# xmlyqing00/V-FloodNet

Hardware: AMD Instinct MI355X
Metric: segmented frames/sec at 480p (higher is better)
Workload: dtype f32

## Files before the change

include/vfn_hip.h:

```cpp
#ifndef VFN_HIP_H
#define VFN_HIP_H

#ifdef __cplusplus
extern "C" {
#endif

#define VFN_ABI_VERSION 16
enum { VFN_DESC_CONV = 0, VFN_DESC_STEM = 1, VFN_DESC_BANKSCAN = 2, VFN_DESC_MEMREAD = 3, VFN_DESC_BANK = 4, VFN_DESC_WGRAD = 5,
       VFN_DESC_REFRESH_FILTER = 6, VFN_DESC_REFRESH_EPILOGUE = 7, VFN_DESC_GATHER = 8, VFN_DESC_BANKMATCH = 9,
       VFN_DESC_TRAIN_AUG = 10 };
int vfn_abi_version(void);
int vfn_sizeof_desc(int which);

typedef struct vfn_conv_desc {
    const float* in;
    const float* w;
    const float* scale;
    const float* shift;
    const float* res;
    float* out;
    int N, H, W, Cin, in_ld;
    int Ho, Wo, Cout, cout_pad, out_ld, res_ld;
    int KH, KW, stride, pad;
    int relu_in, relu_out;
    int M;
    int ksplit;
    int split_from;
    int res_mod;
    float* partial;
    int* tile_counters;
    int w_packed;
    int in_lp;
    int out_lp_relu;
    void* out_lp;
    const float* mask;
    int mask_ld;
    int mask_after;
    int w_batch_rows;
    int k_rot;
} vfn_conv_desc;

int vfn_conv_cfg_count(void);
int vfn_conv_cfg_tile(int cfg, int* bm, int* bn);
int vfn_conv_cfg_info(int cfg, int* bm, int* bn, int* wm, int* wn, int* dma);
int vfn_conv_cfg_modes(int cfg);
int vfn_conv_cfg_wk(int cfg);
int vfn_conv_cfg_tpb(int cfg);
#define VFN_CONV_SK_WS_FLOATS (16 * 1024 * 1024)
#define VFN_CONV_SK_MAX_TILES 16384
int vfn_conv_cfg_kind(int cfg);
int vfn_conv_cfg_name(int cfg, char* buf, int n);
int vfn_conv2d_nhwc_f32(const vfn_conv_desc* d, int cfg, void* stream);
int vfn_conv2d_nhwc_bf16(const vfn_conv_desc* d, int cfg, void* stream);
int vfn_conv2d_nhwc_bf16x3(const vfn_conv_desc* d, int cfg, void* stream);

int vfn_winograd_tiles(int N, int H, int W);
int vfn_winograd_input_f32(const float* x, int N, int H, int W, int C, int ld_x, int relu, float* V, int rows_pad, void* stream);
int vfn_winograd_output_f32(const float* Mb, int rows_pad, int N, int H, int W, int Cout, const float* scale, const float* shift,
                            const float* res, int res_ld, int res_mod, int relu_out, float* out, int out_ld, void* stream);
int vfn_winograd_output_masked_f32(const float* Mb, int rows_pad, int N, int H, int W, int Cout, const float* res, int res_ld,
                                   const float* mask, int mask_ld, int mask_after, float* out, int out_ld, void* stream);
int vfn_winograd_gemm_f32(const float* V, const float* U, float* Mb, int comps, int rows_pad, int C, int Cout, int cout_pad, int cfg,
                          int wgs, void* stream);
int vfn_conv1x1_persistent_f32(const vfn_conv_desc* d, int cfg, int wgs, void* stream);
int vfn_winograd_input_bf16(const float* x, int N, int H, int W, int C, int ld_x, int relu, void* V, int rows_pad, void* stream);
int vfn_winograd_gemm_bf16(const void* V, const void* U, float* Mb, int comps, int rows_pad, int C, int Cout, int cout_pad, int cfg,
                           int wgs, void* stream);
int vfn_winograd_gy_f32(const float* gy, int N, int H, int W, int C, int ld, float* Z, int rows_pad, void* stream);
int vfn_winograd_dw_f32(const float* dU, int Cout, int Cin, const float* rowscale, float* dw, int accumulate, void* stream);

typedef struct vfn_stem_desc {
    const float* frame;
    const float* mask;
    const float* w;
    const float* scale;
    const float* shift;
    float* out;
    float mean[3];
    float std[3];
    int N, cin;
    int H0, W0;
    int pad_top, pad_left;
    int Hp, Wp;
    int Ho, Wo;
} vfn_stem_desc;

int vfn_stem_conv7x7_f32(const vfn_stem_desc* d, void* stream);
int vfn_maxpool3x3s2_nhwc_f32(const float* in, float* out, int N, int H, int W, int C, void* stream);

int vfn_upsample2x_add_nhwc_f32(const float* s, const float* pm, float* out, int N, int h, int w, int C,
                                int s_bcast, void* stream);
int vfn_upsample2x_add_lp_nhwc_f32(const float* s, const float* pm, float* out, void* out_lp, int lp_relu,
// ... 310 lines not shown
```

v-floodnet_amd/_lib.py:

```python
import ctypes as C
import os

import torch

_HERE = os.path.dirname(os.path.abspath(__file__))
LIB_PATH = os.environ.get('VFN_LIB_PATH') or os.path.join(_HERE, 'libvfn_hip.so')

_lib = None

c_fp = C.c_void_p


class ConvDesc(C.Structure):
    _fields_ = [('inp', c_fp), ('w', c_fp), ('scale', c_fp), ('shift', c_fp), ('res', c_fp), ('out', c_fp),
                ('N', C.c_int), ('H', C.c_int), ('W', C.c_int), ('Cin', C.c_int), ('in_ld', C.c_int),
                ('Ho', C.c_int), ('Wo', C.c_int), ('Cout', C.c_int), ('cout_pad', C.c_int),
                ('out_ld', C.c_int), ('res_ld', C.c_int),
                ('KH', C.c_int), ('KW', C.c_int), ('stride', C.c_int), ('pad', C.c_int),
                ('relu_in', C.c_int), ('relu_out', C.c_int), ('M', C.c_int), ('ksplit', C.c_int),
                ('split_from', C.c_int), ('res_mod', C.c_int), ('partial', c_fp), ('tile_counters', c_fp),
                ('w_packed', C.c_int), ('in_lp', C.c_int), ('out_lp_relu', C.c_int), ('out_lp', c_fp), ('mask', c_fp), ('mask_ld', C.c_int), ('mask_after', C.c_int), ('w_batch_rows', C.c_int), ('k_rot', C.c_int)]


class WgradDesc(C.Structure):
# ... 58 lines not shown
class BankDesc(C.Structure):
    _fields_ = [('bank_k', c_fp), ('bank_v', c_fp), ('info', c_fp),
                ('scratch_k', c_fp), ('scratch_v', c_fp), ('scratch_info', c_fp),
                ('bank_len', c_fp), ('bank_len_rw', c_fp), ('bank_knorm', c_fp), ('bank_vnorm', c_fp),
                ('match_idx', c_fp), ('match_corr', c_fp), ('new_k', c_fp), ('new_knorm', c_fp), ('new_vnorm', c_fp),
                ('app_pos', c_fp), ('keep_dst', c_fp), ('plan', c_fp), ('stats', c_fp),
                ('stride_k', C.c_longlong), ('stride_v', C.c_longlong), ('stride_info', C.c_longlong),
                ('stride_n', C.c_longlong), ('stride_new', C.c_longlong),
                ('class_budget', C.c_double),
                ('thres_close', C.c_float), ('update_rate', C.c_float), ('new_hit_init', C.c_float),
                ('frame_idx', C.c_int), ('ld_new', C.c_int), ('voff', C.c_int), ('HW', C.c_int),
                ('obj_n', C.c_int), ('cap', C.c_int), ('rm_class', C.c_int), ('rm_request', C.c_int)]


class TrainAugFrame(C.Structure):
    _fields_ = [('m', C.c_double * 6), ('brightness', C.c_float), ('contrast', C.c_float), ('saturation', C.c_float),
                ('hue_shift', C.c_int), ('order', C.c_int * 4),
                ('flip', C.c_int), ('jitter', C.c_int), ('affine', C.c_int), ('nearest_tables', C.c_int),
                ('win_i', C.c_int), ('win_j', C.c_int), ('win_h', C.c_int), ('win_w', C.c_int)]


TRAIN_AUG_MAX_T, TRAIN_AUG_MAX_SIDE, TRAIN_AUG_MAX_OUT, TRAIN_AUG_MAX_OBJ = 16, 8192, 4096, 11


class TrainAugDesc(C.Structure):
    _fields_ = [('src', c_fp), ('mask', c_fp), ('jit', c_fp), ('lsum', c_fp), ('win_img', c_fp), ('win_mask', c_fp),
                ('aff_xtab', c_fp), ('aff_ytab', c_fp), ('hpass', c_fp), ('kx_bounds', c_fp), ('kx', c_fp),
                ('ky_bounds', c_fp), ('ky', c_fp), ('nx', c_fp), ('ny', c_fp), ('frames', c_fp), ('masks', c_fp),
                ('H', C.c_int), ('W', C.c_int), ('T', C.c_int), ('S', C.c_int), ('ksize_x', C.c_int), ('ksize_y', C.c_int),
                ('obj_n', C.c_int), ('obj_list', C.c_int * (TRAIN_AUG_MAX_OBJ - 1)),
                ('frame', TrainAugFrame * TRAIN_AUG_MAX_T)]


ABI_VERSION = 16
DESC_IDS = {0: ConvDesc, 1: StemDesc, 2: BankScanDesc, 3: MemReadDesc, 4: BankDesc, 5: WgradDesc, 6: RefreshFilter, 7: RefreshEpilogue, 8: GatherEntry, 9: BankMatchDesc, 10: TrainAugDesc}


def lib():
    global _lib
    if _lib is None:
        if not os.path.isfile(LIB_PATH):
            raise RuntimeError(
                f'{LIB_PATH} not found: build the HIP kernels first '
                '(python -c "import __graft_entry__ as g; g.build()" or make -C v-floodnet_amd/csrc)')
        L = C.CDLL(LIB_PATH)
        L.vfn_abi_version.restype = C.c_int
        if L.vfn_abi_version() != ABI_VERSION:
            raise RuntimeError(f'{LIB_PATH} has ABI version {L.vfn_abi_version()}, this package expects {ABI_VERSION} '
                               '(descriptor layouts differ): rebuild it (make -C v-floodnet_amd/csrc)')
        L.vfn_sizeof_desc.restype = C.c_int
        for which, cls in DESC_IDS.items():
            if L.vfn_sizeof_desc(which) != C.sizeof(cls):
                raise RuntimeError(f'{LIB_PATH}: sizeof({cls.__name__}) is {L.vfn_sizeof_desc(which)} in the library, '
                                   f'{C.sizeof(cls)} in this binding: rebuild it (make -C v-floodnet_amd/csrc)')
        _declare(L)
        _lib = L
    return _lib


def _declare(L):
    i, f, p = C.c_int, C.c_float, C.c_void_p
    L.vfn_abi_version.restype = i
    L.vfn_conv_cfg_count.restype = i
    L.vfn_conv_cfg_tile.argtypes = [i, C.POINTER(i), C.POINTER(i)]
    L.vfn_conv_cfg_info.argtypes = [i] + [C.POINTER(i)] * 5
    L.vfn_conv_cfg_wk.argtypes = [i]
    L.vfn_conv_cfg_wk.restype = i
# ... 35 lines not shown
_ll = C.c_longlong
SIGNATURES = {
    'vfn_maxpool3x3s2_nhwc_f32': [_p, _p, _i, _i, _i, _i, _p],
    'vfn_upsample2x_add_nhwc_f32': [_p, _p, _p, _i, _i, _i, _i, _i, _p],
    'vfn_upsample2x_add_lp_nhwc_f32': [_p, _p, _p, _p, _i, _i, _i, _i, _i, _i, _p],
    'vfn_rough_uncertainty_f32': [_p, _p, _p, _p, _i, _i, _i, _p],
    'vfn_transpose_taps_f32': [_p, _i, _i, _i, _i, _i, _i, _i, _i, _i, _i, _i, _p, _p, _i, _p],
    'vfn_dilate2_f32': [_p, _p, _i, _i, _i, _i, _i, _i, _p],
    'vfn_bn_param_grads_f32': [_p, _p, _p, _p, _p, _i, _i, _p, _i, _p, _p, _p],
    'vfn_bn_param_grads_acc_f32': [_p, _p, _p, _p, _p, _i, _i, _p, _i, _p, _p, _i, _p, _p],
    'vfn_maxpool3x3s2_backward_f32': [_p, _p, _p, _i, _i, _i, _i, _p, _i, _p],
    'vfn_softmax_cols_f32': [_p, _i, _i, _i, _f, _p, _p],
    'vfn_softmax_cols_backward_f32': [_p, _p, _i, _i, _i, _f, _p, _p],
    'vfn_adamw_f32': [_p, _p, _p, _p, _ll, C.c_double, C.c_double, C.c_double, C.c_double, C.c_double, _i, _p],
    'vfn_colsum_f32': [_p, _i, _i, _i, _p, _i, _p, _p],
    'vfn_colsum_acc_f32': [_p, _i, _i, _i, _p, _i, _p, _i, _p, _p],
    'vfn_upsample2x_add_backward_f32': [_p, _p, _p, _i, _i, _i, _i, _i, _p],
    'vfn_tail_grad_o_f32': [_p, _p, _p, _p, _p, _p, _i, _i, _i, _i, _i, _i, _i, _p],
    'vfn_segment_loss_f32': [_p, _p, _i, _i, _i, _f, _p, _p, _p, _p],
    'vfn_segment_uncertainty_backward_f32': [_p, _i, _i, _i, _p, _p, _p, _p, _p, _p],
    'vfn_tail_split_f32': [_p, _p, _p, _p, _p, _p, _p, _i, _i, _p],
    'vfn_local_stats_backward_f32': [_p] * 13 + [_i, _i, _i, _i, _p],
    'vfn_local_hpass_f32': [_p, _p, _p, _p, _p, _i, _i, _i, _i, _p],
    'vfn_local_vpass_f32': [_p, _p, _p, _p, _p, _i, _i, _i, _i, _p],
    'vfn_local_stats_f32': [_p, _p, _p, _p, _i, _i, _i, _i, _p],
    'vfn_pred2_gather_f32': [_p, _p, _p, _i, _i, _i, _i, _p],
    'vfn_final_logits_f32': [_p, _p, _p, _p, _p, _i, _i, _i, _i, _i, _i, _i, _p],
    'vfn_bank_scan_finish': [_p, _i, _i, _i, _i, _p, _p, _p, _p, _p],
    'vfn_row_norms': [_p, _ll, _i, _i, _p, _i, _i, _p, _p, _ll, _p],
    'vfn_scatter_mean_f32': [_p, _ll, _ll, _p, _i, _p, _ll, _ll, _i, _p],
    'vfn_winograd_tiles': [_i, _i, _i],
    'vfn_winograd_input_f32': [_p, _i, _i, _i, _i, _i, _i, _p, _i, _p],
    'vfn_winograd_output_f32': [_p, _i, _i, _i, _i, _i, _p, _p, _p, _i, _i, _i, _p, _i, _p],
    'vfn_winograd_gy_f32': [_p, _i, _i, _i, _i, _i, _p, _i, _p],
    'vfn_winograd_gemm_f32': [_p, _p, _p, _i, _i, _i, _i, _i, _i, _i, _p],
    'vfn_conv1x1_persistent_f32': [_p, _i, _i, _p],
    'vfn_winograd_input_bf16': [_p, _i, _i, _i, _i, _i, _i, _p, _i, _p],
    'vfn_winograd_gemm_bf16': [_p, _p, _p, _i, _i, _i, _i, _i, _i, _i, _p],
    'vfn_winograd_dw_f32': [_p, _i, _i, _p, _p, _i, _p],
    'vfn_winograd_output_masked_f32': [_p, _i, _i, _i, _i, _i, _p, _i, _p, _i, _i, _p, _i, _p],
    'vfn_scatter_mean_checked_f32': [_p, _ll, _ll, _p, _ll, _i, _p, _ll, _ll, _i, _ll, _p, _p],
    'vfn_resize_bicubic_f32': [_p, _p, _i, _i, _i, _i, _i, _p],
    'vfn_resize_nearest_f32': [_p, _p, _i, _i, _i, _i, _i, _p],
    'vfn_softmax_objects_f32': [_p, _p, _i, _i, _p],
    'vfn_resize_argmax_u8': [_p, _p, _i, _i, _i, _i, _i, _p],
    'vfn_postprocess_pred_u8': [_p, _i, _i, _p],
    'vfn_postprocess_pred_device_u8': [_p, _p, _p, _i, _i, _p],
    'vfn_to_tensor_u8': [_p, _p, _i, _i, _p],
    'vfn_overlay_u8': [_p, _p, _p, _p, _p, _i, _i, C.c_double, C.c_double, _p],
    'vfn_segment_uncertainty_f32': [_p, _i, _i, _i, _p, _p, _p],
    'vfn_jpeg_entropy_decode': [_p, _ll, _p, _ll, _p, _p],
    'vfn_jpeg_idct_u8': [_p, _p, _p, _i, _i, _i, _p],
    'vfn_jpeg_to_tensor_f32': [_p, _p, _p, _i, _i, _i, _i, _i, _i, _i, _p, _p, _p],
    'vfn_png_sizes': [_i, _i, _i, C.POINTER(_ll), C.POINTER(_ll)],
    'vfn_png_deflate_u8': [_p, _i, _i, _i, _p, _p, _p, _p],
    'vfn_png_unfilter_sizes': [_i, _i, _i, C.POINTER(_i), C.POINTER(_ll)],
    'vfn_png_unfilter_u8': [_p, _i, _i, _i, _p, _p, _p, _p],
    'vfn_png_to_tensor_f32': [_p, _i, _i, _i, _i, _p, _p, _p, _p],
    'vfn_refresh_elems_per_block': [],
    'vfn_refresh_filters_f32': [_p, _i, _i, _p],
    'vfn_refresh_epilogues_f32': [_p, _i, _p],
    'vfn_gather_strided_f32': [_p, _i, _i, _p, _p],
    'vfn_ln_stem_f32': [_p, _p, _p, _p, _p, _i, _i, _i, _i, _i, _i, _i, _p],
    'vfn_ln_dwconv_f32': [_p, _p, _p, _p, _p, _i, _i, _i, _i, _i, _i, _i, _i, _i, _i, _i, _i, _p],
    'vfn_ln_se_gate_f32': [_p, _f, _p, _p, _p, _p, _p, _i, _i, _i, _p],
    'vfn_ln_scale_cols_f32': [_p, _p, _p, _i, _i, _p],
# ... 77 lines not shown
```

v-floodnet_amd/csrc/conv_winograd.hip:

```cpp
#include "common.h"
#include "conv_internal.h"
#include "../../include/vfn_hip.h"

namespace {

__device__ __forceinline__ void bt6(const f32x4 (&v)[6], f32x4 (&t)[6]) {
    t[0] = 4.f * v[0] - 5.f * v[2] + v[4];
    t[1] = -4.f * (v[1] + v[2]) + v[3] + v[4];
    t[2] = 4.f * (v[1] - v[2]) - v[3] + v[4];
    t[3] = -2.f * v[1] - v[2] + 2.f * v[3] + v[4];
    t[4] = 2.f * v[1] - v[2] - 2.f * v[3] + v[4];
    t[5] = 4.f * v[1] - 5.f * v[3] + v[5];
}

template <bool LPOUT = false>
__global__ __launch_bounds__(256)
void winograd_input_kernel(const float* __restrict__ x, int N, int H, int W, int C, int ld_x, int relu, float* __restrict__ V,
                           int rows_pad) {
    const int th = (H + 3) / 4, tw = (W + 3) / 4;
    const int c4n = C / 4;
    const long long total = (long long)N * th * tw * c4n;
    const __amdgpu_buffer_rsrc_t rx = __builtin_amdgcn_make_buffer_rsrc(const_cast<float*>(x), 0, (int)((size_t)N * H * W * ld_x * 4), 0x00020000);
    const float floor_ = relu ? 0.f : -INFINITY;
    for (long long i = vfn_xcd_block(blockIdx.x, gridDim.x) * (long long)blockDim.x + threadIdx.x; i < total; i += (long long)gridDim.x * blockDim.x) {
// ... 106 lines not shown
        for (int b = 0; b < 4; ++b) {
            f32x4 col[6], y[4];
#pragma unroll
            for (int a = 0; a < 6; ++a) col[a] = t[a][b];
            at6(col, y);
#pragma unroll
            for (int a = 0; a < 4; ++a) {
                f32x4 v;
#pragma unroll
                for (int e = 0; e < 4; ++e) v[e] = y[a][e] * sc[e] + sh[e];
                if constexpr (MASK) {
                    if (!mask_after) {
#pragma unroll
                        for (int e = 0; e < 4; ++e) v[e] = mk[a][b][e] > 0.f ? v[e] : 0.f;
                    }
                }
                v += rv[a][b];
                if constexpr (MASK) {
                    if (mask_after) {
#pragma unroll
                        for (int e = 0; e < 4; ++e) v[e] = mk[a][b][e] > 0.f ? v[e] : 0.f;
                    }
                }
#pragma unroll
                for (int e = 0; e < 4; ++e) v[e] = vfn_floor_nan(v[e], floor_);
                const int row = rowi[a][b];
                __builtin_amdgcn_raw_buffer_store_b128(__builtin_bit_cast(__attribute__((ext_vector_type(4))) unsigned, v), ro,
                                                       row >= 0 ? (row * out_ld + c4 * 4) * 4 : 0x7ffffff0, 0, 0);
            }
        }
    }
}

__device__ __forceinline__ void a6(const f32x4 (&v)[4], f32x4 (&z)[6]) {
    const f32x4 e = v[0] + v[2], o = v[1] + v[3];
    const f32x4 e4 = v[0] + 4.f * v[2], o8 = 2.f * v[1] + 8.f * v[3];
    z[0] = v[0];
    z[1] = e + o;
    z[2] = e - o;
    z[3] = e4 + o8;
    z[4] = e4 - o8;
    z[5] = v[3];
}

__global__ __launch_bounds__(256)
void winograd_gy_kernel(const float* __restrict__ gy, int N, int H, int W, int C, int ld, float* __restrict__ Z, int rows_pad) {
    const int th = (H + 3) / 4, tw = (W + 3) / 4;
    const int c4n = C / 4;
    const long long total = (long long)N * th * tw * c4n;
    for (long long i = vfn_xcd_block(blockIdx.x, gridDim.x) * (long long)blockDim.x + threadIdx.x; i < total; i += (long long)gridDim.x * blockDim.x) {
        const int c4 = (int)(i % c4n);
        const int tile = (int)(i / c4n);
        const int tx = tile % tw, ty = (tile / tw) % th, n = tile / (tw * th);
        f32x4 t[6][4];
#pragma unroll
        for (int b = 0; b < 4; ++b) {
            f32x4 col[4], z[6];
            const int xx = 4 * tx + b;
#pragma unroll
            for (int a = 0; a < 4; ++a) {
                const int yy = 4 * ty + a;
                f32x4 v = {0.f, 0.f, 0.f, 0.f};
                if (yy < H && xx < W) v = *reinterpret_cast<const f32x4*>(gy + ((size_t)(n * H + yy) * W + xx) * ld + c4 * 4);
                col[a] = v;
            }
            a6(col, z);
// ... 292 lines not shown
    wino_gemm_args p = a;
    p.mtiles = (a.rows_pad + BM - 1) / BM;
    p.ntiles = (a.Cout + BN - 1) / BN;
    const int total = p.comps * p.mtiles * p.ntiles;
    int grid = wgs > 0 ? wgs : 512;
    if (grid > total) grid = total;
    grid = (grid + 7) / 8 * 8;
    hipLaunchKernelGGL((wino_gemm_kernel<BM, BN, WM, WN, PD, CONV, LP>), dim3(grid), dim3(WM * WN * 64), lds, s, p);
    return vfn_check_launch();
}

constexpr int kWinoTile[4][4] = {{128, 128, 4, 2}, {64, 128, 2, 4}, {128, 64, 4, 2}, {64, 64, 2, 2}};
constexpr int kWinoCfgs = 8;

template <bool CONV, bool LP>
int launch_wino_cfg(const wino_gemm_args& a, int cfg, int wgs, hipStream_t s) {
    return vfn_dispatch<kWinoCfgs>(cfg, [&](auto id) -> int {
        constexpr int c = decltype(id)::value;
        constexpr const int* t = kWinoTile[c & 3];
        return launch_wino_gemm<t[0], t[1], t[2], t[3], 1 + (c >> 2), CONV, LP>(a, wgs, s);
    });
}

inline bool tensors_fit_32bit(int N, int H, int W, int ld, int res_ld, int mask_ld, int res_mod) {
    const long long px = (long long)N * H * W;
    return px * ld * 4 < 0x7fffff00LL && (res_mod > 0 ? (long long)res_mod : px) * res_ld * 4 < 0x7fffff00LL && px * mask_ld * 4 < 0x7fffff00LL;
}

inline int grid_of(long long total) {
    long long b = (total + 255) / 256;
    return (int)(b < 16384 ? (b ? b : 1) : 16384);
}

}

extern "C" int vfn_winograd_tiles(int N, int H, int W) { return N * ((H + 3) / 4) * ((W + 3) / 4); }

extern "C" int vfn_winograd_input_f32(const float* x, int N, int H, int W, int C, int ld_x, int relu, float* V, int rows_pad, void* stream) {
    if (!x || !V || N < 1 || H < 1 || W < 1 || C < 4 || C % 4 || ld_x < C || ld_x % 4 || rows_pad < vfn_winograd_tiles(N, H, W)) return VFN_ERR_ARG;
    const long long total = (long long)vfn_winograd_tiles(N, H, W) * (C / 4);
    if (!tensors_fit_32bit(N, H, W, ld_x, 0, 0, 0)) return VFN_ERR_ARG;
    hipLaunchKernelGGL(winograd_input_kernel<false>, dim3(grid_of(total)), dim3(256), 0, (hipStream_t)stream, x, N, H, W, C, ld_x, relu, V, rows_pad);
    return vfn_check_launch();
}

extern "C" int vfn_winograd_output_f32(const float* Mb, int rows_pad, int N, int H, int W, int Cout, const float* scale, const float* shift,
                                       const float* res, int res_ld, int res_mod, int relu_out, float* out, int out_ld, void* stream) {
    if (!Mb || !out || N < 1 || H < 1 || W < 1 || Cout < 4 || Cout % 4 || out_ld < Cout || out_ld % 4 || (res && res_ld % 4) ||
        rows_pad < vfn_winograd_tiles(N, H, W)) return VFN_ERR_ARG;
    const long long total = (long long)vfn_winograd_tiles(N, H, W) * (Cout / 4);
    if (!tensors_fit_32bit(N, H, W, out_ld, res ? res_ld : 0, 0, res_mod)) return VFN_ERR_ARG;
    hipLaunchKernelGGL(winograd_output_kernel<false>, dim3(grid_of(total)), dim3(256), 0, (hipStream_t)stream, Mb, rows_pad, N, H, W, Cout, scale, shift,
                       res, res_ld, res_mod, relu_out, out, out_ld, (const float*)nullptr, 0, 0);
    return vfn_check_launch();
}

extern "C" int vfn_winograd_output_masked_f32(const float* Mb, int rows_pad, int N, int H, int W, int Cout, const float* res, int res_ld,
                                              const float* mask, int mask_ld, int mask_after, float* out, int out_ld, void* stream) {
    if (!Mb || !out || N < 1 || H < 1 || W < 1 || Cout < 4 || Cout % 4 || out_ld < Cout || out_ld % 4 || (res && res_ld % 4) ||
        (mask && mask_ld % 4) || rows_pad < vfn_winograd_tiles(N, H, W)) return VFN_ERR_ARG;
    const long long total = (long long)vfn_winograd_tiles(N, H, W) * (Cout / 4);
    if (!tensors_fit_32bit(N, H, W, out_ld, res ? res_ld : 0, mask ? mask_ld : 0, 0)) return VFN_ERR_ARG;
    if (mask)
        hipLaunchKernelGGL(winograd_output_kernel<true>, dim3(grid_of(total)), dim3(256), 0, (hipStream_t)stream, Mb, rows_pad, N, H, W, Cout,
                           (const float*)nullptr, (const float*)nullptr, res, res_ld, 0, 0, out, out_ld, mask, mask_ld, mask_after);
    else
        hipLaunchKernelGGL(winograd_output_kernel<false>, dim3(grid_of(total)), dim3(256), 0, (hipStream_t)stream, Mb, rows_pad, N, H, W, Cout,
                           (const float*)nullptr, (const float*)nullptr, res, res_ld, 0, 0, out, out_ld, (const float*)nullptr, 0, 0);
    return vfn_check_launch();
}

extern "C" int vfn_winograd_gy_f32(const float* gy, int N, int H, int W, int C, int ld, float* Z, int rows_pad, void* stream) {
    if (!gy || !Z || N < 1 || H < 1 || W < 1 || C < 4 || C % 4 || ld < C || ld % 4 || rows_pad < vfn_winograd_tiles(N, H, W)) return VFN_ERR_ARG;
    const long long total = (long long)vfn_winograd_tiles(N, H, W) * (C / 4);
    hipLaunchKernelGGL(winograd_gy_kernel, dim3(grid_of(total)), dim3(256), 0, (hipStream_t)stream, gy, N, H, W, C, ld, Z, rows_pad);
    return vfn_check_launch();
}

extern "C" int vfn_winograd_dw_f32(const float* dU, int Cout, int Cin, const float* rowscale, float* dw, int accumulate, void* stream) {
    if (!dU || !dw || Cout < 1 || Cin < 4 || Cin % 4) return VFN_ERR_ARG;
    hipLaunchKernelGGL(winograd_dw_kernel, dim3(grid_of((long long)Cout * (Cin / 4))), dim3(256), 0, (hipStream_t)stream, dU, Cout, Cin, rowscale,
                       dw, accumulate);
    return vfn_check_launch();
}

extern "C" int vfn_winograd_gemm_f32(const float* V, const float* U, float* Mb, int comps, int rows_pad, int C, int Cout, int cout_pad, int cfg,
                                     int wgs, void* stream) {
// ... 42 lines not shown
```

v-floodnet_amd/engine.py:

```python
import math
import os

import torch

from . import _lib, ops, weights as W
from ._lib import ptr, stream, check, MemReadDesc, BankScanDesc
from .feature_bank import pick_nsplit, pick_scan_slices, MAX_SPLIT, MAX_SPLIT_SCAN, QT_SCAN, DK, DV

_CFG_EFF = {(128, 128): 1.00, (128, 64): 0.95, (64, 128): 0.95, (64, 64): 0.86, (32, 64): 0.74,
            (64, 32): 0.74, (128, 32): 0.80, (256, 128): 0.97}
_CFG_TILES = None
_TUNED = {}
_TUNED_PATH = __import__('os').path.join(__import__('os').path.dirname(__import__('os').path.abspath(__file__)),
                                         'tuned_gfx950.json')
_TUNED_BF16 = {}
_TUNED_BF16_PATH = _TUNED_PATH.replace('tuned_gfx950.json', 'tuned_gfx950_bf16.json')
_TUNED_BF16X3 = {}
_TUNED_BF16X3_PATH = _TUNED_PATH.replace('tuned_gfx950.json', 'tuned_gfx950_bf16x3.json')
_TABLES = (_TUNED, _TUNED_BF16, _TUNED_BF16X3)
_TABLE_PATHS = (_TUNED_PATH, _TUNED_BF16_PATH, _TUNED_BF16X3_PATH)


def _load_tuned():
    import json
# ... 8 lines not shown
            for k, v in json.load(open(path)).items():
                t = (int(v[0]), int(v[1]), int(v[2]) if len(v) > 2 else 0)
                table[tuple(int(x) for x in k.split(','))] = t + tuple(int(x) for x in v[3:6]) if len(v) >= 6 else t


def save_tuned(path=None, mode=0):
    import json
    table = _TABLES[mode]
    with open(path or _TABLE_PATHS[mode], 'w') as f:
        json.dump({','.join(str(x) for x in k): list(v) for k, v in sorted(table.items())}, f, indent=0)


_load_tuned()


def pad_divide_by(h, w, d=16):
    new_h = h + d - h % d if h % d > 0 else h
    new_w = w + d - w % d if w % d > 0 else w
    lh = int((new_h - h) / 2)
    uh = int(new_h - h) - lh
    lw = int((new_w - w) / 2)
    uw = int(new_w - w) - lw
    return (lw, uw, lh, uh), new_h, new_w


WS_FLOATS = 16 * 1024 * 1024
_WINOGRAD_TRAIN = os.environ.get('VFN_WINOGRAD_TRAIN', '1') == '1'
_BATCH_MEMREAD = os.environ.get('VFN_TRAIN_BATCH_MEMREAD', '1') == '1'
MAX_GROUP = 16
_TRAIN_SLOTS = int(os.environ.get('VFN_TRAIN_SLOTS', 2))
_WINOGRAD = os.environ.get('VFN_WINOGRAD', '1')
_WINOGRAD_LP = os.environ.get('VFN_WINOGRAD_LP', '1') == '1'
_WINOGRAD_MIN_M = int(os.environ.get('VFN_WINOGRAD_MIN_M', 10000))
_WINO_TABLE = {}
_WINO_TABLE_BF16 = {}
_WINO_PATH = os.path.join(os.path.dirname(os.path.abspath(__file__)), 'wino_gfx950.json')
if os.environ.get('VFN_IGNORE_TUNED') != '1':
    for _path, _tab in ((_WINO_PATH, _WINO_TABLE), (_WINO_PATH.replace('.json', '_bf16.json'), _WINO_TABLE_BF16)):
        if os.path.isfile(_path):
            _tab.update({tuple(int(x) for x in k.split(',')): int(v) for k, v in __import__('json').load(open(_path)).items()})
_INLAUNCH_SPLITK = __import__('os').environ.get('VFN_INLAUNCH_SPLITK', '1') == '1'


def _tiles():
    global _CFG_TILES
    if _CFG_TILES is None:
        _CFG_TILES = ops.conv_cfg_tiles()
    return _CFG_TILES


def apply_choice(desc, choice, ws, counters=None):
    cfg, ks, split_from = choice[:3]
    if ks > 1 and (desc.out_ld % 4 or (desc.res and desc.res_ld % 4)):
        ks, split_from = 1, 0
    if cfg >= ops.PCONV_CFG0 and not ops.pconv_eligible(desc, 0):
        fb = tuple(choice[3:6]) if len(choice) >= 6 else choose_cfg(desc.M, desc.Cout, desc.KH * desc.KW * desc.Cin, 0, use_table=False)
        return apply_choice(desc, fb, ws, counters)
    if cfg >= ops.WINO_GEMM_CFG0:
        ops.set_splitk(desc, 1, None)
        return cfg
    if ops.conv_cfg_kind(cfg) == 2:
        if counters is None or ws is None or ws.numel() < ops.SK_WS_FLOATS:
            ws, counters = ops.streamk_scratch(ws.device if ws is not None else torch.device('cuda', torch.cuda.current_device()))
        ops.set_streamk(desc, ws, counters)
        return cfg
    if ks > 1:
# ... 429 lines not shown
        bf = self.eng.layer_mode(name)
        lp = bf == 2
        if self.eng.mixed:
            f32_out = True
        if ((bf == 0 or (bf == 1 and _WINOGRAD_LP and not self.keep_acts and layer.cin % 64 == 0)) and in_ld is None and
                (_WINOGRAD_TRAIN or not self.keep_acts) and x.shape[-1] == layer.cin and self.eng.use_winograd(layer, N * H * Wd, bf)):
            return self._conv_winograd(lst, layer, x, out, N, H, Wd, res, relu_in, relu_out, name, out_ld, res_mod, bf)
        d = ops.make_conv_desc(x, layer.w, layer.cout, layer.k, layer.k, layer.stride, layer.pad, out,
                               layer.scale, layer.shift, res, relu_in, relu_out,
                               cin=layer.cin, in_ld=in_ld if in_ld is not None else x.shape[-1],
                               out_ld=out_ld, N=N, H=H, W=Wd)
        d.res_mod = int(res_mod)
        if lp and in_ld is None and layer.cin % 32 == 0 and self.has_lp(x, relu_in):
            d.inp, d.in_lp, d.relu_in = ptr(self.lp_twin(x)), 1, 0
        if lp and lp_out and layer.cout % 32 == 0 and d.out_ld % 32 == 0:
            d.out_lp, d.out_lp_relu = ptr(self.lp_twin(out)), int(lp_out == 'relu')
            self._lp_state[(out.data_ptr(), tuple(out.shape))] = (lp_out == 'relu')
            if not f32_out:
                d.out = None
        else:
            self._lp_state.pop((out.data_ptr(), tuple(out.shape)), None)
        K = layer.k * layer.k * layer.cin
        if bf == 1 and layer.cin % 64:
            bf = 2
        if bf:
            ops.use_packed_weights(d, layer.w_lp(bf))
        choice = choose_cfg(d.M, layer.cout, K, bf)
        if choice[1] > 1 and (d.out_ld % 4 or (res is not None and d.res_ld % 4)):
            choice = (choice[0], 1, 0)
        cfg = apply_choice(d, choice, self._ws_cur, self._cnt_cur)
        lst.append(Launch(ops.conv2d_launch, (d, cfg, bf), f'{name}[{d.M}x{layer.cout}x{K}]', 2.0 * d.M * layer.cout * K))
        return out

    def _conv_winograd(self, lst, layer, x, out, N, H, Wd, res, relu_in, relu_out, name, out_ld, res_mod, bf=0):
        rows = ops.winograd_rows(N, H, Wd)
        key = id(self._ws_cur)
        need_v, need_m = 36 * rows * layer.cin, 36 * rows * layer.cout
        V, Mb = self._wino.get(key, (None, None))
        if V is None or V.numel() < need_v or Mb.numel() < need_m:
            dev = self.eng.device
            V = torch.zeros(max(need_v, V.numel() if V is not None else 0), device=dev)
            Mb = torch.empty(max(need_m, Mb.numel() if Mb is not None else 0), device=dev)
            self._wino[key] = (V, Mb)
        Mb = Mb[:need_m].view(36 * rows, layer.cout)
        if bf == 1:
            V = V.view(torch.bfloat16)[:need_v].view(36 * rows, layer.cin)
            U = layer.w_wino_bf16()
        else:
            V = V[:need_v].view(36 * rows, layer.cin)
            U = layer.w_wino()
        lst.append(Launch(ops.winograd_input, (x, V, rows, relu_in, N, H, Wd, layer.cin, x.shape[-1]), name + '.wino_in'))
        dg = ops.make_winograd_gemm_desc(V, U, Mb, rows, layer.cin, layer.cout)
        if bf:
            choice = _TABLES[bf].get((dg.M, layer.cout, layer.cin))
            if choice is None or choice[0] < ops.WINO_GEMM_CFG0:
                tc = 5 if rows % 64 == 0 and layer.cout >= 128 and rows >= 1024 else 3
                choice = (ops.wino_gemm_cfg(tc, 512), 1, 0)
        else:
            choice = choose_cfg(dg.M, layer.cout, layer.cin, 0)
        cfg = apply_choice(dg, choice, self._ws_cur, self._cnt_cur)
        lst.append(Launch(ops.conv2d_launch, (dg, cfg, bf), f'{name}.wino_gemm[{dg.M}x{layer.cout}x{layer.cin}]', 2.0 * dg.M * layer.cout * layer.cin))
        self._lp_state.pop((out.data_ptr(), tuple(out.shape)), None)
        lst.append(Launch(ops.winograd_output, (Mb, rows, out, N, H, Wd, layer.cout, layer.scale, layer.shift, res,
                                                res.shape[-1] if res is not None else 0, res_mod, relu_out,
                                                out_ld if out_ld is not None else out.shape[-1]), name + '.wino_out'))
        return out

    def _trunk(self, lst, enc, bufs, N, prefix, acts=None):
        x = bufs['x4']
        lst.append(Launch(ops.maxpool3x3s2, (bufs['r1'], x), prefix + '.maxpool'))
        H, Wd = self.h4, self.w4
        for lname in ('res2', 'res3', 'res4'):
            blocks = enc[lname]
            lb = bufs[lname]
            for bi, blk in enumerate(blocks):
                s = blk['conv2'].stride
                Ho, Wo = H // s, Wd // s
                t1 = lb['t1a'] if (s == 2) else lb['t1']
                t2, ds_buf = lb['t2'], lb['ds']
                if self.keep_acts:
                    t1, t2 = torch.empty_like(t1), torch.empty_like(lb['t2'])
                    ds_buf = torch.empty_like(lb['ds'])
                nm = f'{prefix}.{lname}.{bi}'
                self._conv(lst, blk['conv1'], x, t1, N, H, Wd, relu_out=True, name=nm + '.conv1', lp_out='plain', f32_out=False)
                self._conv(lst, blk['conv2'], t1, t2, N, H, Wd, relu_out=True, name=nm + '.conv2', lp_out='plain',
                           f32_out=False)
                if 'down' in blk:
                    self._conv(lst, blk['down'], x, ds_buf, N, H, Wd, name=nm + '.down')
                    idn = ds_buf
                else:
                    idn = x
                out = lb['out'] if bi == len(blocks) - 1 else lb['o'][bi % 2]
                if self.keep_acts and bi != len(blocks) - 1:
                    out = torch.empty_like(out)
                self._conv(lst, blk['conv3'], t2, out, N, Ho, Wo, res=idn, relu_out=True, name=nm + '.conv3',
                           lp_out='plain')
                if self.keep_acts and acts is not None:
                    acts[(lname, bi)] = dict(x=x, t1=t1, t2=t2, ds=ds_buf if 'down' in blk else None, out=out, stride=s, H=H, W=Wd)
                x = out
                H, Wd = Ho, Wo
        return x

    def _resblock(self, lst, rb, x, t, out, N, H, Wd, name):
        self._conv(lst, rb['conv1'], x, t, N, H, Wd, relu_in=True, name=name + '.conv1', lp_out='relu', f32_out=False)
        self._conv(lst, rb['conv2'], t, out, N, H, Wd, res=x, relu_in=True, name=name + '.conv2')
        return out

    def _build(self):
        e = self.eng
        K = self.obj_n
        for qs in self.qsets:
            qs.build()
        self._ws_cur, self._cnt_cur = self.ws, self.cnt
        self.stem_m = ops.make_stem_desc(self.frame_in, self.mask_in, e.stem_m_w, e.stem_m_scale, e.stem_m_shift,
                                         self.m['r1'], e.mean, e.std, K, self.H0, self.W0, self.pad, self.Hp, self.Wp)
        self.mem.append(Launch(ops.stem_launch, (self.stem_m,), 'encoder_m.stem',
                               2.0 * K * self.h2 * self.w2 * 64 * 245))
        r4m = self._trunk(self.mem, e.enc_m, self.m, K, 'encoder_m', acts=self.acts_m)
        self._conv(self.mem, e.keyval, r4m, self.kv_m, K, self.h16, self.w16, name='keyval')

    def conv_flops(self, which):
        return sum(l.flops for l in getattr(self, which))


class QuerySet:

    def __init__(self, plan, nq=2):
        self.plan = plan
        self.nq = nq
        p = plan
        f = lambda *s_: torch.empty(*s_, device=p.eng.device, dtype=torch.float32)
        self.frames = f(nq, 3, p.H0, p.W0)
        self.q = p._trunk_buffers(nq)
        self.kv_q = f(nq, p.HW, DK + DV)
        self.fm_q = f(nq, p.h16, p.w16, 256)
        self.s8 = [f(nq, p.h8, p.w8, 256) for _ in range(3)]
# ... 708 lines not shown
```

v-floodnet_amd/ops.py:

```python
import ctypes as C
import os

import torch

from . import _lib
from ._lib import ptr, stream, check, ConvDesc


_cfg_tiles = None


def conv_cfg_tiles():
    global _cfg_tiles
    if _cfg_tiles is None:
        L = _lib.lib()
        out = []
        for c in range(L.vfn_conv_cfg_count()):
            bm, bn = C.c_int(), C.c_int()
            L.vfn_conv_cfg_tile(c, C.byref(bm), C.byref(bn))
            out.append((bm.value, bn.value))
        _cfg_tiles = tuple(out)
    return _cfg_tiles


# ... 264 lines not shown
    assert tuple(w.shape[2:]) == (3, 3)
    g = w.detach().double().cpu()
    U = torch.einsum('ia,ocab,jb->ijoc', _WINO_G, g, _WINO_G)
    cp = (cout + 255) // 256 * 256
    out = torch.zeros(36, cp, cin, dtype=torch.float32)
    out[:, :cout] = U.reshape(36, cout, cin).float()
    return out.reshape(36 * cp, cin).contiguous()


def winograd_rows(N, H, W):
    t = N * ((H + 3) // 4) * ((W + 3) // 4)
    return (t + WINO_ROW_MULT - 1) // WINO_ROW_MULT * WINO_ROW_MULT


def pack_winograd_weight_bf16(w):
    return pack_winograd_weight(w).to(torch.bfloat16).contiguous()


def winograd_input(x, V, rows_pad, relu, N=None, H=None, W=None, cin=None, ld_x=None):
    if N is None:
        N, H, W = x.shape[0], x.shape[1], x.shape[2]
    cin = cin if cin is not None else x.shape[-1]
    ld_x = ld_x if ld_x is not None else x.shape[-1]
    if V.dtype == torch.bfloat16:
        check(_lib.lib().vfn_winograd_input_bf16(ptr(x), N, H, W, cin, ld_x, int(relu), ptr(V), rows_pad, stream()), 'vfn_winograd_input_bf16')
        return
    check(_lib.lib().vfn_winograd_input_f32(ptr(x), N, H, W, cin, ld_x, int(relu), ptr(V), rows_pad, stream()), 'vfn_winograd_input_f32')


def winograd_output(Mb, rows_pad, out, N, H, W, cout, scale, shift, res, res_ld, res_mod, relu_out, out_ld=None):
    check(_lib.lib().vfn_winograd_output_f32(ptr(Mb), rows_pad, N, H, W, cout, ptr(scale), ptr(shift), ptr(res), int(res_ld), int(res_mod),
                                             int(relu_out), ptr(out), out_ld if out_ld is not None else out.shape[-1], stream()),
          'vfn_winograd_output_f32')


def make_winograd_gemm_desc(V, U, Mb, rows_pad, cin, cout):
    d = make_conv_desc(V, U, cout, 1, 1, 1, 0, Mb, None, None, None, False, False, cin=cin, in_ld=cin, out_ld=cout, N=1, H=1, W=36 * rows_pad)
    d.cout_pad = U.shape[0] // 36
    d.w_batch_rows = rows_pad
    d.k_rot = _WINO_KROT
    return d


def winograd_gemm(V, U, Mb, rows_pad, cin, cout, cfg=0, wgs=0, comps=36):
    check(_lib.lib().vfn_winograd_gemm_f32(ptr(V), ptr(U), ptr(Mb), comps, rows_pad, cin, cout, U.shape[0] // comps, int(cfg), int(wgs), stream()),
          'vfn_winograd_gemm_f32')


def conv2d_winograd(x, w, scale=None, shift=None, res=None, relu_in=False, relu_out=False, cfg=2, res_mod=0):
    N, H, W, cin = x.shape
    cout = w.shape[0]
    rows = winograd_rows(N, H, W)
    U = pack_winograd_weight(w).to(x.device)
    V = torch.empty(36 * rows, cin, device=x.device, dtype=torch.float32)
    Mb = torch.empty(36 * rows, cout, device=x.device, dtype=torch.float32)
    out = torch.empty(N, H, W, cout, device=x.device, dtype=torch.float32)
    if rows > vfn_winograd_tiles(N, H, W):
        V.view(36, rows, cin)[:, vfn_winograd_tiles(N, H, W):].zero_()
    winograd_input(x, V, rows, relu_in)
    d = make_winograd_gemm_desc(V, U, Mb, rows, cin, cout)
    if conv_cfg_kind(cfg) == 2:
        set_streamk(d, *streamk_scratch(x.device))
    conv2d_launch(d, cfg, 0)
    winograd_output(Mb, rows, out, N, H, W, cout, scale, shift, res, res.shape[-1] if res is not None else 0, res_mod, relu_out)
    return out

# ... 402 lines not shown
```

Before: 160.7.

## Fuse Winograd output and next-layer input transforms inside residual blocks

Adds a kernel that reads conv1's Winograd-domain GEMM result and applies the inverse transform, BN scale/shift and ReLU. It stages the spatial tile plus a one-tile halo ring in LDS, then applies the forward input transform for conv2 and writes V directly. This skips writing the intermediate activation to global memory and reading it back, and removes one launch per residual block. The cost is recomputing halo tiles (or larger blocks), heavy LDS and register use, and a fused path that only covers f32 Winograd layers with channels a multiple of 32.

```diff
diff --git a/include/vfn_hip.h b/include/vfn_hip.h
--- a/include/vfn_hip.h
+++ b/include/vfn_hip.h
@@ -5,7 +5,7 @@
 extern "C" {
 #endif
 
-#define VFN_ABI_VERSION 16
+#define VFN_ABI_VERSION 17
 enum { VFN_DESC_CONV = 0, VFN_DESC_STEM = 1, VFN_DESC_BANKSCAN = 2, VFN_DESC_MEMREAD = 3, VFN_DESC_BANK = 4, VFN_DESC_WGRAD = 5,
        VFN_DESC_REFRESH_FILTER = 6, VFN_DESC_REFRESH_EPILOGUE = 7, VFN_DESC_GATHER = 8, VFN_DESC_BANKMATCH = 9,
        VFN_DESC_TRAIN_AUG = 10 };
@@ -58,6 +58,8 @@
 int vfn_winograd_input_f32(const float* x, int N, int H, int W, int C, int ld_x, int relu, float* V, int rows_pad, void* stream);
 int vfn_winograd_output_f32(const float* Mb, int rows_pad, int N, int H, int W, int Cout, const float* scale, const float* shift,
                             const float* res, int res_ld, int res_mod, int relu_out, float* out, int out_ld, void* stream);
+int vfn_winograd_out_in_f32(const float* Mb, int rows_pad, int N, int H, int W, int C, const float* scale, const float* shift,
+                            float* V, void* stream);
 int vfn_winograd_output_masked_f32(const float* Mb, int rows_pad, int N, int H, int W, int Cout, const float* res, int res_ld,
                                    const float* mask, int mask_ld, int mask_after, float* out, int out_ld, void* stream);
 int vfn_winograd_gemm_f32(const float* V, const float* U, float* Mb, int comps, int rows_pad, int C, int Cout, int cout_pad, int cfg,
diff --git a/v-floodnet_amd/_lib.py b/v-floodnet_amd/_lib.py
--- a/v-floodnet_amd/_lib.py
+++ b/v-floodnet_amd/_lib.py
@@ -114,7 +114,7 @@
                 ('frame', TrainAugFrame * TRAIN_AUG_MAX_T)]
 
 
-ABI_VERSION = 16
+ABI_VERSION = 17
 DESC_IDS = {0: ConvDesc, 1: StemDesc, 2: BankScanDesc, 3: MemReadDesc, 4: BankDesc, 5: WgradDesc, 6: RefreshFilter, 7: RefreshEpilogue, 8: GatherEntry, 9: BankMatchDesc, 10: TrainAugDesc}
 
 
@@ -216,6 +216,7 @@
     'vfn_winograd_tiles': [_i, _i, _i],
     'vfn_winograd_input_f32': [_p, _i, _i, _i, _i, _i, _i, _p, _i, _p],
     'vfn_winograd_output_f32': [_p, _i, _i, _i, _i, _i, _p, _p, _p, _i, _i, _i, _p, _i, _p],
+    'vfn_winograd_out_in_f32': [_p, _i, _i, _i, _i, _i, _p, _p, _p, _p],
     'vfn_winograd_gy_f32': [_p, _i, _i, _i, _i, _i, _p, _i, _p],
     'vfn_winograd_gemm_f32': [_p, _p, _p, _i, _i, _i, _i, _i, _i, _i, _p],
     'vfn_conv1x1_persistent_f32': [_p, _i, _i, _p],
diff --git a/v-floodnet_amd/csrc/conv_winograd.hip b/v-floodnet_amd/csrc/conv_winograd.hip
--- a/v-floodnet_amd/csrc/conv_winograd.hip
+++ b/v-floodnet_amd/csrc/conv_winograd.hip
@@ -162,6 +162,118 @@
     }
 }
 
+template <int kFuseTH, int kFuseTW, bool ONEPASS>
+__global__ __launch_bounds__((kFuseTH * kFuseTW + (ONEPASS ? 2 * (kFuseTH + kFuseTW) + 4 : 0)) * 8)
+void winograd_out_in_kernel(const float* __restrict__ Mb, int rows_pad, int N, int H, int W, int C, const float* __restrict__ scale,
+                            const float* __restrict__ shift, float* __restrict__ V, int xmap) {
+    constexpr int kFuseC4 = 8;
+    constexpr int kFusePH = 4 * kFuseTH + 2, kFusePW = 4 * kFuseTW + 2;
+    constexpr int kFuseRing = 2 * (kFuseTH + kFuseTW) + 4;
+    constexpr int TILES = kFuseTH * kFuseTW;
+    constexpr int STEP = ONEPASS ? TILES + kFuseRing : TILES;
+    extern __shared__ __attribute__((aligned(16))) char smem[];
+    f32x4* sr = reinterpret_cast<f32x4*>(smem);
+    const int th = (H + 3) / 4, tw = (W + 3) / 4;
+    const int bh = (th + kFuseTH - 1) / kFuseTH, bw = (tw + kFuseTW - 1) / kFuseTW;
+    const int slices = C / (4 * kFuseC4);
+    int slice, bt;
+    if (xmap) {
+        const int spx = slices >> 3, xcd = blockIdx.x & 7, loc = blockIdx.x >> 3;
+        slice = xcd * spx + loc % spx, bt = loc / spx;
+    } else {
+        const unsigned blk = vfn_xcd_block(blockIdx.x, gridDim.x);
+        slice = (int)(blk % slices), bt = (int)(blk / slices);
+    }
+    const int bx = bt % bw, by = (bt / bw) % bh, n = bt / (bw * bh);
+    const int tid = threadIdx.x;
+    const size_t bytes = (size_t)36 * rows_pad * C * 4;
+    const __amdgpu_buffer_rsrc_t rm = __builtin_amdgcn_make_buffer_rsrc(const_cast<float*>(Mb), 0, (int)bytes, 0x00020000);
+    const __amdgpu_buffer_rsrc_t rv = __builtin_amdgcn_make_buffer_rsrc(V, 0, (int)bytes, 0x00020000);
+    const int comp = rows_pad * C * 4;
+    {
+        const int c4l = tid % kFuseC4;
+        const int c = (slice * kFuseC4 + c4l) * 4;
+        f32x4 sc = {1.f, 1.f, 1.f, 1.f}, sh = {0.f, 0.f, 0.f, 0.f};
+        if (scale) sc = *reinterpret_cast<const f32x4*>(scale + c);
+        if (shift) sh = *reinterpret_cast<const f32x4*>(shift + c);
+        for (int k = tid / kFuseC4; k < TILES + kFuseRing; k += STEP) {
+            int ly, lx;
+            if (k < TILES) {
+                ly = k / kFuseTW, lx = k % kFuseTW;
+            } else {
+                const int j = k - TILES;
+                if (j < kFuseTW) ly = -1, lx = j;
+                else if (j < 2 * kFuseTW) ly = kFuseTH, lx = j - kFuseTW;
+                else if (j < 2 * kFuseTW + kFuseTH) ly = j - 2 * kFuseTW, lx = -1;
+                else if (j < 2 * (kFuseTW + kFuseTH)) ly = j - 2 * kFuseTW - kFuseTH, lx = kFuseTW;
+                else ly = ((j - 2 * (kFuseTW + kFuseTH)) & 2) ? kFuseTH : -1, lx = ((j - 2 * (kFuseTW + kFuseTH)) & 1) ? kFuseTW : -1;
+            }
+            const int ty = by * kFuseTH + ly, tx = bx * kFuseTW + lx;
+            const bool tile_ok = (unsigned)ty < (unsigned)th && (unsigned)tx < (unsigned)tw;
+            const int base = tile_ok ? (((n * th + ty) * tw + tx) * C + c) * 4 : 0;
+            f32x4 m[6][6];
+#pragma unroll
+            for (int a = 0; a < 6; ++a)
+#pragma unroll
+                for (int b = 0; b < 6; ++b)
+                    m[a][b] = __builtin_bit_cast(f32x4, __builtin_amdgcn_raw_buffer_load_b128(rm, tile_ok ? base + (a * 6 + b) * comp : 0x7ffffff0, 0, 0));
+            f32x4 t[6][4];
+#pragma unroll
+            for (int a = 0; a < 6; ++a) at6(m[a], t[a]);
+#pragma unroll
+            for (int b = 0; b < 4; ++b) {
+                f32x4 col[6], y[4];
+#pragma unroll
+                for (int a = 0; a < 6; ++a) col[a] = t[a][b];
+                at6(col, y);
+                const int xx = 4 * tx + b, px = 1 + 4 * lx + b;
+#pragma unroll
+                for (int a = 0; a < 4; ++a) {
+                    const int yy = 4 * ty + a, py = 1 + 4 * ly + a;
+                    const bool ok = (unsigned)yy < (unsigned)H && (unsigned)xx < (unsigned)W;
+                    f32x4 v;
+#pragma unroll
+                    for (int e = 0; e < 4; ++e) v[e] = y[a][e] * sc[e] + sh[e];
+#pragma unroll
+                    for (int e = 0; e < 4; ++e) v[e] = ok ? vfn_floor_nan(v[e], 0.f) : 0.f;
+                    if ((unsigned)py < (unsigned)kFusePH && (unsigned)px < (unsigned)kFusePW) sr[(py * kFusePW + px) * kFuseC4 + c4l] = v;
+                }
+            }
+        }
+    }
+    __syncthreads();
+    if (tid < TILES * kFuseC4) {
+        const int c4l = tid % kFuseC4, k = tid / kFuseC4;
+        const int ly = k / kFuseTW, lx = k % kFuseTW;
+        const int ty = by * kFuseTH + ly, tx = bx * kFuseTW + lx;
+        const bool tile_ok = ty < th && tx < tw;
+        const int base = tile_ok ? (((n * th + ty) * tw + tx) * C + (slice * kFuseC4 + c4l) * 4) * 4 : 0;
+        f32x4 d[6][6];
+#pragma unroll
+        for (int a = 0; a < 6; ++a)
+#pragma unroll
+            for (int b = 0; b < 6; ++b) d[a][b] = sr[((4 * ly + a) * kFusePW + 4 * lx + b) * kFuseC4 + c4l];
+#pragma unroll
+        for (int b = 0; b < 6; ++b) {
+            f32x4 v[6], t[6];
+#pragma unroll
+            for (int a = 0; a < 6; ++a) v[a] = d[a][b];
+            bt6(v, t);
+#pragma unroll
+            for (int a = 0; a < 6; ++a) d[a][b] = t[a];
+        }
+#pragma unroll
+        for (int a = 0; a < 6; ++a) {
+            f32x4 t[6];
+            bt6(d[a], t);
+#pragma unroll
+            for (int b = 0; b < 6; ++b)
+                __builtin_amdgcn_raw_buffer_store_b128(__builtin_bit_cast(__attribute__((ext_vector_type(4))) unsigned, t[b]), rv,
+                                                       tile_ok ? base + (a * 6 + b) * comp : 0x7ffffff0, 0, 0);
+        }
+    }
+}
+
 __device__ __forceinline__ void a6(const f32x4 (&v)[4], f32x4 (&z)[6]) {
     const f32x4 e = v[0] + v[2], o = v[1] + v[3];
     const f32x4 e4 = v[0] + 4.f * v[2], o8 = 2.f * v[1] + 8.f * v[3];
@@ -520,6 +632,18 @@
     return (int)(b < 16384 ? (b ? b : 1) : 16384);
 }
 
+template <int TH, int TW, bool ONEPASS>
+int launch_out_in(const float* Mb, int rows_pad, int N, int H, int W, int C, const float* scale, const float* shift, float* V, long long blocks,
+                  hipStream_t s) {
+    constexpr size_t lds = (size_t)(4 * TH + 2) * (4 * TW + 2) * 8 * sizeof(f32x4);
+    constexpr int nt = (TH * TW + (ONEPASS ? 2 * (TH + TW) + 4 : 0)) * 8;
+    static const bool lds_ready = vfn_allow_lds(&winograd_out_in_kernel<TH, TW, ONEPASS>, lds);
+    (void)lds_ready;
+    hipLaunchKernelGGL((winograd_out_in_kernel<TH, TW, ONEPASS>), dim3((unsigned)blocks), dim3(nt), lds, s, Mb, rows_pad, N, H, W, C, scale, shift, V,
+                       (C / 32) % 8 == 0 ? 1 : 0);
+    return vfn_check_launch();
+}
+
 }
 
 extern "C" int vfn_winograd_tiles(int N, int H, int W) { return N * ((H + 3) / 4) * ((W + 3) / 4); }
@@ -541,6 +665,17 @@
     hipLaunchKernelGGL(winograd_output_kernel<false>, dim3(grid_of(total)), dim3(256), 0, (hipStream_t)stream, Mb, rows_pad, N, H, W, Cout, scale, shift,
                        res, res_ld, res_mod, relu_out, out, out_ld, (const float*)nullptr, 0, 0);
     return vfn_check_launch();
+}
+
+extern "C" int vfn_winograd_out_in_f32(const float* Mb, int rows_pad, int N, int H, int W, int C, const float* scale, const float* shift,
+                                       float* V, void* stream) {
+    if (!Mb || !V || N < 1 || H < 1 || W < 1 || C < 32 || C % 32 || rows_pad < vfn_winograd_tiles(N, H, W)) return VFN_ERR_ARG;
+    if ((long long)36 * rows_pad * C * 4 >= 0x7fffff00LL) return VFN_ERR_ARG;
+    const int th = (H + 3) / 4, tw = (W + 3) / 4, bw = (tw + 6) / 7;
+    const long long big = (long long)N * ((th + 7) / 8) * bw * (C / 32), small = (long long)N * ((th + 3) / 4) * bw * (C / 32);
+    if (small >= 0x7fffffffLL) return VFN_ERR_ARG;
+    if (big >= 256) return launch_out_in<8, 7, false>(Mb, rows_pad, N, H, W, C, scale, shift, V, big, (hipStream_t)stream);
+    return launch_out_in<4, 7, true>(Mb, rows_pad, N, H, W, C, scale, shift, V, small, (hipStream_t)stream);
 }
 
 extern "C" int vfn_winograd_output_masked_f32(const float* Mb, int rows_pad, int N, int H, int W, int Cout, const float* res, int res_ld,
diff --git a/v-floodnet_amd/engine.py b/v-floodnet_amd/engine.py
--- a/v-floodnet_amd/engine.py
+++ b/v-floodnet_amd/engine.py
@@ -64,6 +64,7 @@
 _WINOGRAD = os.environ.get('VFN_WINOGRAD', '1')
 _WINOGRAD_LP = os.environ.get('VFN_WINOGRAD_LP', '1') == '1'
 _WINOGRAD_MIN_M = int(os.environ.get('VFN_WINOGRAD_MIN_M', 10000))
+_WINOGRAD_FUSED = os.environ.get('VFN_WINOGRAD_FUSED', '1') == '1'
 _WINO_TABLE = {}
 _WINO_TABLE_BF16 = {}
 _WINO_PATH = os.path.join(os.path.dirname(os.path.abspath(__file__)), 'wino_gfx950.json')
@@ -559,24 +560,24 @@
         lst.append(Launch(ops.conv2d_launch, (d, cfg, bf), f'{name}[{d.M}x{layer.cout}x{K}]', 2.0 * d.M * layer.cout * K))
         return out
 
-    def _conv_winograd(self, lst, layer, x, out, N, H, Wd, res, relu_in, relu_out, name, out_ld, res_mod, bf=0):
-        rows = ops.winograd_rows(N, H, Wd)
+    def _wino_scratch(self, rows, cin, cout, bf=0):
         key = id(self._ws_cur)
-        need_v, need_m = 36 * rows * layer.cin, 36 * rows * layer.cout
+        need_v, need_m = 36 * rows * cin, 36 * rows * cout
         V, Mb = self._wino.get(key, (None, None))
         if V is None or V.numel() < need_v or Mb.numel() < need_m:
             dev = self.eng.device
             V = torch.zeros(max(need_v, V.numel() if V is not None else 0), device=dev)
             Mb = torch.empty(max(need_m, Mb.numel() if Mb is not None else 0), device=dev)
             self._wino[key] = (V, Mb)
-        Mb = Mb[:need_m].view(36 * rows, layer.cout)
+        Mb = Mb[:need_m].view(36 * rows, cout)
         if bf == 1:
-            V = V.view(torch.bfloat16)[:need_v].view(36 * rows, layer.cin)
-            U = layer.w_wino_bf16()
+            V = V.view(torch.bfloat16)[:need_v].view(36 * rows, cin)
         else:
-            V = V[:need_v].view(36 * rows, layer.cin)
-            U = layer.w_wino()
-        lst.append(Launch(ops.winograd_input, (x, V, rows, relu_in, N, H, Wd, layer.cin, x.shape[-1]), name + '.wino_in'))
+            V = V[:need_v].view(36 * rows, cin)
+        return V, Mb
+
+    def _wino_gemm(self, lst, layer, V, Mb, rows, name, bf=0):
+        U = layer.w_wino_bf16() if bf == 1 else layer.w_wino()
         dg = ops.make_winograd_gemm_desc(V, U, Mb, rows, layer.cin, layer.cout)
         if bf:
             choice = _TABLES[bf].get((dg.M, layer.cout, layer.cin))
@@ -587,6 +588,12 @@
             choice = choose_cfg(dg.M, layer.cout, layer.cin, 0)
         cfg = apply_choice(dg, choice, self._ws_cur, self._cnt_cur)
         lst.append(Launch(ops.conv2d_launch, (dg, cfg, bf), f'{name}.wino_gemm[{dg.M}x{layer.cout}x{layer.cin}]', 2.0 * dg.M * layer.cout * layer.cin))
+
+    def _conv_winograd(self, lst, layer, x, out, N, H, Wd, res, relu_in, relu_out, name, out_ld, res_mod, bf=0):
+        rows = ops.winograd_rows(N, H, Wd)
+        V, Mb = self._wino_scratch(rows, layer.cin, layer.cout, bf)
+        lst.append(Launch(ops.winograd_input, (x, V, rows, relu_in, N, H, Wd, layer.cin, x.shape[-1]), name + '.wino_in'))
+        self._wino_gemm(lst, layer, V, Mb, rows, name, bf)
         self._lp_state.pop((out.data_ptr(), tuple(out.shape)), None)
         lst.append(Launch(ops.winograd_output, (Mb, rows, out, N, H, Wd, layer.cout, layer.scale, layer.shift, res,
                                                 res.shape[-1] if res is not None else 0, res_mod, relu_out,
@@ -628,7 +635,27 @@
                 H, Wd = Ho, Wo
         return x
 
+    def _resblock_fused(self, rb, x, N, H, Wd, name):
+        c1, c2 = rb['conv1'], rb['conv2']
+        if not _WINOGRAD_FUSED or self.keep_acts or c1.cout != c2.cin or c1.cout % 32 or x.shape[-1] != c1.cin:
+            return False
+        return all(self.eng.layer_mode(f'{name}.{cn}') == 0 and self.eng.use_winograd(rb[cn], N * H * Wd, 0) for cn in ('conv1', 'conv2'))
+
     def _resblock(self, lst, rb, x, t, out, N, H, Wd, name):
+        if self._resblock_fused(rb, x, N, H, Wd, name):
+            c1, c2 = rb['conv1'], rb['conv2']
+            rows = ops.winograd_rows(N, H, Wd)
+            V1, M1 = self._wino_scratch(rows, c1.cin, c1.cout)
+            V2, M2 = self._wino_scratch(rows, c2.cin, c2.cout)
+            lst.append(Launch(ops.winograd_input, (x, V1, rows, True, N, H, Wd, c1.cin, x.shape[-1]), name + '.conv1.wino_in'))
+            self._wino_gemm(lst, c1, V1, M1, rows, name + '.conv1')
+            lst.append(Launch(ops.winograd_out_in, (M1, rows, V2, N, H, Wd, c1.cout, c1.scale, c1.shift), name + '.conv1.wino_out_in'))
+            self._wino_gemm(lst, c2, V2, M2, rows, name + '.conv2')
+            for b in (t, out):
+                self._lp_state.pop((b.data_ptr(), tuple(b.shape)), None)
+            lst.append(Launch(ops.winograd_output, (M2, rows, out, N, H, Wd, c2.cout, c2.scale, c2.shift, x, x.shape[-1], 0, False,
+                                                    out.shape[-1]), name + '.conv2.wino_out'))
+            return out
         self._conv(lst, rb['conv1'], x, t, N, H, Wd, relu_in=True, name=name + '.conv1', lp_out='relu', f32_out=False)
         self._conv(lst, rb['conv2'], t, out, N, H, Wd, res=x, relu_in=True, name=name + '.conv2')
         return out
diff --git a/v-floodnet_amd/ops.py b/v-floodnet_amd/ops.py
--- a/v-floodnet_amd/ops.py
+++ b/v-floodnet_amd/ops.py
@@ -320,6 +320,10 @@
     check(_lib.lib().vfn_winograd_output_f32(ptr(Mb), rows_pad, N, H, W, cout, ptr(scale), ptr(shift), ptr(res), int(res_ld), int(res_mod),
                                              int(relu_out), ptr(out), out_ld if out_ld is not None else out.shape[-1], stream()),
           'vfn_winograd_output_f32')
+
+
+def winograd_out_in(Mb, rows_pad, V, N, H, W, c, scale, shift):
+    check(_lib.lib().vfn_winograd_out_in_f32(ptr(Mb), rows_pad, N, H, W, c, ptr(scale), ptr(shift), ptr(V), stream()), 'vfn_winograd_out_in_f32')
 
 
 def make_winograd_gemm_desc(V, U, Mb, rows_pad, cin, cout):
```

After: 161.3, median of 6. About the same (+0.4%).
